# santiagolmedo/gnn_qot_estimation

Measured on AMD Instinct MI355X. Metric: graphs/sec (train step) on 100-node/400-edge synthetic topologies, batch=1024, higher is better.
Workload: dtype f32; 1 GPU; configs[1]: 2-layer TopologicalGNN (TransformerConv+NNConv) hidden=64, 100-node/400-directed-edge topologies, batch=1024 graphs per GPU, dropout 0.5, SGD momentum 0.9, SmoothL1; CSR build included in every step; graphs_per_gpu=1024, global_batch=1024, distinct_graphs_per_gpu=1024, launch=hip-graph replay, 4 whole steps (fwd+bwd+optimizer each) per graph, steps_per_graph=4, collective_in_graph=False, parallelism=dp1, prime_steps=45, collective_world_size=1, all_reduce_floats=68715

## Files before the change

gnn_qot_estimation_amd/csrc/nnconv_mfma.hip:

```cpp
#include "common.hpp"
#include "mfma_tile.hpp"
#include "nnconv_finalize_dev.hpp"
#include "split_bf16.hpp"

namespace qot {

template <int D, bool TRANSPOSE>
__device__ __forceinline__ void nnconv_gather_tile(
    float* __restrict__ At, const float* __restrict__ x, int ldx, const float* __restrict__ ea,
    const float* __restrict__ w1, const float* __restrict__ b1, const int32_t* __restrict__ rowptr,
    const int32_t* __restrict__ col, const int32_t* __restrict__ eidx, const float* __restrict__ invdeg,
    int64_t tile0, int64_t N, float4& root0, float4& root1) {
    constexpr int K = 2 * D;
    const int sub = threadIdx.x & 7, il = threadIdx.x >> 3;
    const int c0 = 8 * sub;
    const int64_t i = tile0 + il;
    float4 acc0[K + 1], acc1[K + 1];
    root0 = f4zero(); root1 = f4zero();
    int beg = 0, end = 0;
    float srow = 0.f;
    if (i < N) {
        beg = rowptr[i]; end = rowptr[i + 1];
        if (!TRANSPOSE) srow = invdeg[i];
        root0 = ld4(x + i * ldx + c0);
        root1 = ld4(x + i * ldx + c0 + 4);
    }
    const int own = (i < N) ? (int)i : 0;
#define QOT_ACC(FIRSTSLOT, H, X, A) ((FIRSTSLOT) ? scale4((H), (X)) : fma4((H), (X), (A)))
#define QOT_EDGE4(U0, FIRST)                                                                            \
        {                                                                                               \
            float4 xa[4], xb[4];                                                                        \
            float sc[4];                                                                                \
            int jj[4];                                                                                  \
            jj[0] = group8_bcast<U0 + 0>(myj); jj[1] = group8_bcast<U0 + 1>(myj);                       \
            jj[2] = group8_bcast<U0 + 2>(myj); jj[3] = group8_bcast<U0 + 3>(myj);                       \
            sc[0] = group8_bcast<U0 + 0>(mysc); sc[1] = group8_bcast<U0 + 1>(mysc);                     \
            sc[2] = group8_bcast<U0 + 2>(mysc); sc[3] = group8_bcast<U0 + 3>(mysc);                     \
            _Pragma("unroll") for (int u = 0; u < 4; ++u) {                                             \
                const float* xr = x + (int64_t)jj[u] * ldx + c0;                                        \
                xa[u] = ld4(xr);                                                                        \
                xb[u] = ld4(xr + 4);                                                                    \
            }                                                                                           \
            _Pragma("unroll") for (int kk = 0; kk < K; ++kk) {                                          \
                const float h0 = group8_bcast<U0 + 0>(myh[kk]), h1 = group8_bcast<U0 + 1>(myh[kk]);     \
                acc0[kk] = QOT_ACC(FIRST, h0, xa[0], acc0[kk]); acc1[kk] = QOT_ACC(FIRST, h0, xb[0], acc1[kk]); \
                acc0[kk] = fma4(h1, xa[1], acc0[kk]); acc1[kk] = fma4(h1, xb[1], acc1[kk]);             \
            }                                                                                           \
            acc0[K] = QOT_ACC(FIRST, sc[0], xa[0], acc0[K]); acc1[K] = QOT_ACC(FIRST, sc[0], xb[0], acc1[K]); \
            acc0[K] = fma4(sc[1], xa[1], acc0[K]); acc1[K] = fma4(sc[1], xb[1], acc1[K]);               \
             \
             \
            if (cnt > U0 + 2) {                                                                         \
                _Pragma("unroll") for (int kk = 0; kk < K; ++kk) {                                      \
                    const float h2 = group8_bcast<U0 + 2>(myh[kk]), h3 = group8_bcast<U0 + 3>(myh[kk]); \
                    acc0[kk] = fma4(h2, xa[2], acc0[kk]); acc1[kk] = fma4(h2, xb[2], acc1[kk]);         \
                    acc0[kk] = fma4(h3, xa[3], acc0[kk]); acc1[kk] = fma4(h3, xb[3], acc1[kk]);         \
                }                                                                                       \
                _Pragma("unroll") for (int u = 2; u < 4; ++u) {                                         \
                    acc0[K] = fma4(sc[u], xa[u], acc0[K]);                                              \
                    acc1[K] = fma4(sc[u], xb[u], acc1[K]);                                              \
                }                                                                                       \
            }                                                                                           \
        }
#define QOT_FWD_BATCH(FIRST)                                                                            \
    {                                                                                                   \
        const int p = base + sub;                                                                       \
        int myj = own;                                                                                  \
        float myh[K], mysc = 0.f;                                                                       \
        _Pragma("unroll") for (int kk = 0; kk < K; ++kk) myh[kk] = 0.f;                                 \
        if (p < end) {                                                                                  \
            myj = col[p];                                                                               \
            const int64_t e = (int64_t)eidx[p];                                                         \
            float ee[D];                                                                                \
            _Pragma("unroll") for (int d = 0; d < D; ++d) ee[d] = ea[e * D + d];                        \
            mysc = TRANSPOSE ? invdeg[myj] : srow;                                                      \
            _Pragma("unroll") for (int kk = 0; kk < K; ++kk) {                                          \
                float h = b1[kk];                                                                       \
                _Pragma("unroll") for (int d = 0; d < D; ++d) h = fmaf(w1[kk * D + d], ee[d], h);       \
                myh[kk] = fmaxf(h, 0.f) * mysc;                                                         \
            }                                                                                           \
        }                                                                                               \
        const int cnt = (end - base < 8) ? end - base : 8;                                              \
        QOT_EDGE4(0, FIRST)                                                                             \
        if (cnt > 4) QOT_EDGE4(4, false)                                                                \
    }
    int base = beg;
    QOT_FWD_BATCH(true)
    for (base = beg + 8; base < end; base += 8) QOT_FWD_BATCH(false)
#undef QOT_FWD_BATCH
#undef QOT_EDGE4
#undef QOT_ACC
    float4* At4 = reinterpret_cast<float4*>(At);
#pragma unroll
    for (int kk = 0; kk <= K; ++kk) {
        const int g = kk * 8 + sub;
        At4[at4_slot(g, 0, il)] = make_float4(acc0[kk].x, acc0[kk].z, acc1[kk].x, acc1[kk].z);
        At4[at4_slot(g, 1, il)] = make_float4(acc0[kk].y, acc0[kk].w, acc1[kk].y, acc1[kk].w);
    }
}

template <int D, bool TRANSPOSE, bool SPLIT = false>
__global__ __launch_bounds__(256, 2) void nnconv_mfma64_kernel(
    const float* __restrict__ x, int ldx, const float* __restrict__ ea, const float* __restrict__ w1,
    const float* __restrict__ b1, const int32_t* __restrict__ rowptr, const int32_t* __restrict__ col,
    const int32_t* __restrict__ eidx, const float* __restrict__ invdeg, const float* __restrict__ Wp,
    const float* __restrict__ bias, float* __restrict__ out, int64_t N, ActParams act,
    const u32x4* __restrict__ Ws = nullptr, int64_t ws_planes = 0) {
    static_assert(!SPLIT || !TRANSPOSE, "split form: forward only");
    constexpr int K = 2 * D;
    constexpr int KM = (K + 1) * 64;
    constexpr int GM = KM / 16;
    constexpr int CH = 4;
    __shared__ __attribute__((aligned(16))) float At[KM * 32];
    const int64_t ntiles = (N + 31) / 32;
    const float bz = bias ? bias[((threadIdx.x >> 6) & 1) * 32 + (threadIdx.x & 31)] : 0.f;
    const uint64_t drop_step = (act.enabled && act.thr16) ? (uint64_t)act.step[0] : 0;
#pragma unroll 1
    for (int64_t it = 0;; ++it) {
    const int64_t tile = xcd_tile(it, ntiles);
    if (tile < 0) break;
    const int64_t tile0 = tile * 32;
    float4 root0, root1;
    nnconv_gather_tile<D, TRANSPOSE>(At, x, ldx, ea, w1, b1, rowptr, col, eidx, invdeg, tile0, N, root0, root1);
    const float4* At4 = reinterpret_cast<const float4*>(At);
    const int lane = threadIdx.x & 63, wave = threadIdx.x >> 6;
    const int nh = wave & 1, kh = wave >> 1;
    const int r31 = lane & 31, hi = lane >> 5;
    f32x16 c;
#pragma unroll
    for (int r = 0; r < 16; ++r) c[r] = 0.f;
    if constexpr (SPLIT) {
        constexpr int ST = (K + 2) * 64 / 16;
        constexpr int SM = GM / 2;
        constexpr int SC = 2;
        constexpr int NCS = SM / SC;
        constexpr int NBS = 3;
        static_assert(GM % 4 == 0, "chunking");
        const u32x4* wsn = Ws + (int64_t)nh * ST * 64 + lane;
        const u32x4* wsp = wsn + (int64_t)kh * SM * 64;
        const u32x4* rsp = wsn + (int64_t)(2 * SM + 2 * kh) * 64;
        asm volatile("" : "+v"(rsp));
        Bf3 rbs[2];
#pragma unroll
        for (int u = 0; u < 2; ++u) rbs[u] = load_split_b(rsp + u * 64, ws_planes);
        Bf3 sb[NBS][SC];
#pragma unroll
        for (int q = 0; q < NBS - 1; ++q)
#pragma unroll
            for (int u = 0; u < SC; ++u) sb[q][u] = load_split_b(wsp + (q * SC + u) * 64, ws_planes);
        lds_barrier();
        int ch = 0;
#pragma unroll 1
        for (; ch + NBS <= NCS; ch += NBS) {
#pragma unroll
            for (int q = 0; q < NBS; ++q) {
                if (ch + q + NBS - 1 < NCS) {
#pragma unroll
                    for (int u = 0; u < SC; ++u)
                        sb[(q + NBS - 1) % NBS][u] = load_split_b(wsp + ((ch + q + NBS - 1) * SC + u) * 64, ws_planes);
                }
#pragma unroll
                for (int u = 0; u < SC; ++u) c = mfma_split_step(At4, kh * GM + 2 * ((ch + q) * SC + u), hi, r31, sb[q][u], c);
            }
        }
#pragma unroll
        for (int q = 0; q < NBS - 1; ++q) {
            if (ch + q < NCS) {
#pragma unroll
                for (int u = 0; u < SC; ++u) c = mfma_split_step(At4, kh * GM + 2 * ((ch + q) * SC + u), hi, r31, sb[q][u], c);
            }
        }
        lds_barrier();
        {
            float4* At4w = reinterpret_cast<float4*>(At);
            const int sub = threadIdx.x & 7, il = threadIdx.x >> 3;
            At4w[at4_slot(sub, 0, il)] = make_float4(root0.x, root0.z, root1.x, root1.z);
            At4w[at4_slot(sub, 1, il)] = make_float4(root0.y, root0.w, root1.y, root1.w);
        }
        __syncthreads();
#pragma unroll
        for (int u = 0; u < 2; ++u) c = mfma_split_step(At4, kh * 4 + 2 * u, hi, r31, rbs[u], c);
    } else {
    const float4* wpn = reinterpret_cast<const float4*>(Wp) + (int64_t)nh * (2 * GM + 8) * 64 + lane;
    const float4* wp = wpn + (int64_t)kh * GM * 64;
    const float4* rbp = wpn + (int64_t)(2 * GM + kh * 4) * 64;
    asm volatile("" : "+v"(rbp));
    float4 rb[4];
#pragma unroll
    for (int u = 0; u < 4; ++u) rb[u] = rbp[u * 64];
    constexpr int NCH = GM / CH;
    constexpr int NB = 4;
    float4 bb[NB][CH];
#pragma unroll
    for (int q = 0; q < NB - 1; ++q)
#pragma unroll
        for (int u = 0; u < CH; ++u) bb[q][u] = wp[(q * CH + u) * 64];
    lds_barrier();
    int ch = 0;
#pragma unroll 1
    for (; ch + NB <= NCH; ch += NB) {
#pragma unroll
        for (int q = 0; q < NB; ++q) {
            if (ch + q + NB - 1 < NCH) {
#pragma unroll
                for (int u = 0; u < CH; ++u) bb[(q + NB - 1) % NB][u] = wp[((ch + q + NB - 1) * CH + u) * 64];
            }
#pragma unroll
            for (int u = 0; u < CH; ++u) c = mfma_group(At4, kh * GM + (ch + q) * CH + u, hi, r31, bb[q][u], c);
        }
    }
#pragma unroll
    for (int q = 0; q < NB - 1; ++q) {
        if (ch + q < NCH) {
#pragma unroll
            for (int u = 0; u < CH; ++u) c = mfma_group(At4, kh * GM + (ch + q) * CH + u, hi, r31, bb[q][u], c);
        }
    }
    lds_barrier();
    {
        float4* At4 = reinterpret_cast<float4*>(At);
        const int sub = threadIdx.x & 7, il = threadIdx.x >> 3;
        At4[at4_slot(sub, 0, il)] = make_float4(root0.x, root0.z, root1.x, root1.z);
        At4[at4_slot(sub, 1, il)] = make_float4(root0.y, root0.w, root1.y, root1.w);
    }
    __syncthreads();
#pragma unroll
    for (int u = 0; u < 4; ++u) c = mfma_group(At4, kh * 4 + u, hi, r31, rb[u], c);
    }
    float* red = At + 64 * 32;
    if (kh) {
#pragma unroll
        for (int r = 0; r < 8; ++r) red[((2 + nh) * 8 + r) * 64 + lane] = c[r];
    } else {
#pragma unroll
        for (int r = 0; r < 8; ++r) red[(nh * 8 + r) * 64 + lane] = c[8 + r];
    }
    lds_barrier();
    {
        const int colg = nh * 32 + r31;
        float v[8];
        if (kh) {
#pragma unroll
            for (int r = 0; r < 8; ++r) v[r] = c[8 + r] + red[(nh * 8 + r) * 64 + lane] + bz;
        } else {
#pragma unroll
            for (int r = 0; r < 8; ++r) v[r] = c[r] + red[((2 + nh) * 8 + r) * 64 + lane] + bz;
        }
        uint32_t zlo[8], zhi[8];
        const bool drop = act.enabled && act.thr16;
        if (drop) {
            const int jq = r31 & 3;
            uint32_t mylo[2], myhi[2];
#pragma unroll
            for (int t = 0; t < 2; ++t) {
                const int rr = kh * 8 + 2 * jq + t;
                const int row = (rr & 3) + 8 * (rr >> 2) + 4 * hi;
                const uint64_t flat = (uint64_t)((tile0 + row) * 64 + colg);
                const uint64_t z = act_hash64(act.seed, drop_step, flat >> 2);
                mylo[t] = (uint32_t)z; myhi[t] = (uint32_t)(z >> 32);
            }
#define QOT_ZSHARE(S)                                                                                   \
            zlo[2 * (S)] = __builtin_amdgcn_update_dpp(0, mylo[0], (S) * 0x55, 0xF, 0xF, true);         \
            zhi[2 * (S)] = __builtin_amdgcn_update_dpp(0, myhi[0], (S) * 0x55, 0xF, 0xF, true);         \
            zlo[2 * (S) + 1] = __builtin_amdgcn_update_dpp(0, mylo[1], (S) * 0x55, 0xF, 0xF, true);     \
            zhi[2 * (S) + 1] = __builtin_amdgcn_update_dpp(0, myhi[1], (S) * 0x55, 0xF, 0xF, true);
            QOT_ZSHARE(0) QOT_ZSHARE(1) QOT_ZSHARE(2) QOT_ZSHARE(3)
#undef QOT_ZSHARE
        }
#pragma unroll
        for (int r = 0; r < 8; ++r) {
            const int rr = kh * 8 + r;
            const int row = (rr & 3) + 8 * (rr >> 2) + 4 * hi;
            const int64_t i = tile0 + row;
            float y = v[r];
            if (act.enabled) {
                y = y > 0.f ? y : act.slope * y;
                if (drop) {
                    const uint64_t z = ((uint64_t)zhi[r] << 32) | zlo[r];
                    const bool keep = ((uint32_t)(z >> (16 * (colg & 3))) & 0xFFFFu) >= act.thr16;
                    y = keep ? y * act.keep_scale : 0.f;
                }
            }
            if (i < N) out[i * 64 + colg] = y;
        }
    }
    lds_barrier();
    }
}


template <int D, bool SPLIT>
__global__ __launch_bounds__(512, 2) void nnconv_adjoint_dw64_kernel(
    const float* __restrict__ g, int ldg, const float* __restrict__ xf, int ldx, const float* __restrict__ ea,
    const float* __restrict__ w1, const float* __restrict__ b1, const int32_t* __restrict__ rowptr_t,
    const int32_t* __restrict__ col_t, const int32_t* __restrict__ eid_t, const float* __restrict__ invdeg,
    const float* __restrict__ Wp, float* __restrict__ gx, float* __restrict__ slabs, int64_t N) {
    constexpr int K = 2 * D;
    constexpr int KT = (K + 2) * 64;
    constexpr int GQ = KT / 8 / 4;
    constexpr int MB = KT / 32;
    constexpr int TPW = MB * 2 / 8;
    static_assert(GQ % 4 == 0 || GQ % 5 == 0, "chunking");
    constexpr int CH = (GQ % 4 == 0) ? 4 : 5;
    __shared__ __attribute__((aligned(16))) float Ut[KT * 32];
    __shared__ __attribute__((aligned(16))) float red[8 * 3 * 4 * 64];
    __shared__ __attribute__((aligned(16))) float xs[32 * 64];
    float4* Ut4 = reinterpret_cast<float4*>(Ut);
    const int lane = threadIdx.x & 63, wave = threadIdx.x >> 6;
    const int r31 = lane & 31, hi = lane >> 5;
    const int nh = wave & 1, kq = wave >> 1;
    const int ah = wave & 1, mb0 = wave >> 1;
    const int64_t ntiles = (N + 31) / 32;

    f32x16 dw[TPW];
#pragma unroll
    for (int t = 0; t < TPW; ++t)
#pragma unroll
        for (int r = 0; r < 16; ++r) dw[t][r] = 0.f;
    int dwoff[4];
    {
        const int kcol = mb0 * 32 + r31;
        const int gg = kcol >> 3, within = kcol & 7;
        const int base0 = ((2 * gg + (within & 1)) * 32) * 4 + (within >> 1);
        const int m = gg & 7;
#pragma unroll
        for (int b = 0; b < 4; ++b) dwoff[b] = base0 + ((((b ^ (m >> 1)) << 1) | (hi ^ (m & 1))) << 2);
    }
    const float4* wp = reinterpret_cast<const float4*>(Wp) + ((int64_t)nh * (KT / 8) + kq * GQ) * 64 + lane;

#pragma unroll 1
    for (int64_t it = 0;; ++it) {
        const int64_t tile = xcd_tile(it, ntiles);
        if (tile < 0) break;
        const int64_t tile0 = tile * 32;
        float4 xown;
        {
            const int64_t j = tile0 + (threadIdx.x >> 4);
            xown = (j < N) ? ld4(xf + j * ldx + 4 * (threadIdx.x & 15)) : f4zero();
        }
        {
            const int sub = threadIdx.x & 15, il = threadIdx.x >> 4;
            const int c0 = 4 * sub;
            const int64_t j = tile0 + il;
            float4 acc[K + 2];
            acc[K + 1] = f4zero();
            int beg = 0, end = 0;
            if (j < N) { beg = rowptr_t[j]; end = rowptr_t[j + 1]; acc[K + 1] = ld4(g + j * ldg + c0); }
            const int own = (j < N) ? (int)j : 0;
#define QOT_ADJ_EDGE(U)                                                                                  \
                {                                                                                        \
                    const int64_t i = (int64_t)row16_bcast<U>(myi);                                      \
                    gr[(U) & 3] = ld4(g + i * ldg + c0);                                                 \
                    sc[(U) & 3] = row16_bcast<U>(mysc);                                                  \
                }
#define QOT_ADJ_FMA(U, FIRSTSLOT)                                                                        \
                {                                                                                        \
                    _Pragma("unroll") for (int kk = 0; kk < K; ++kk)                                     \
                        acc[kk] = (FIRSTSLOT) ? scale4(row16_bcast<U>(myh[kk]), gr[(U) & 3])             \
                                              : fma4(row16_bcast<U>(myh[kk]), gr[(U) & 3], acc[kk]);     \
                    acc[K] = (FIRSTSLOT) ? scale4(sc[(U) & 3], gr[(U) & 3]) : fma4(sc[(U) & 3], gr[(U) & 3], acc[K]); \
                }
#define QOT_ADJ_EDGE4(U0, FIRST)                                                                         \
                {                                                                                        \
                    float4 gr[4];                                                                        \
                    float sc[4];                                                                         \
                    QOT_ADJ_EDGE(U0) QOT_ADJ_EDGE(U0 + 1) QOT_ADJ_EDGE(U0 + 2) QOT_ADJ_EDGE(U0 + 3)      \
                    QOT_ADJ_FMA(U0, FIRST) QOT_ADJ_FMA(U0 + 1, false)                                    \
                     \
                     \
                    if (cnt > U0 + 2) { QOT_ADJ_FMA(U0 + 2, false) QOT_ADJ_FMA(U0 + 3, false) }          \
                }
#define QOT_ADJ_BATCH(FIRST)                                                                             \
            {                                                                                            \
                const int p = base + sub;                                                                \
                int myi = own;                                                                           \
                float myh[K], mysc = 0.f;                                                                \
                _Pragma("unroll") for (int kk = 0; kk < K; ++kk) myh[kk] = 0.f;                          \
                if (p < end) {                                                                           \
                    myi = col_t[p];                                                                      \
                    const int64_t e = (int64_t)eid_t[p];                                                 \
                    float ee[D];                                                                         \
                    _Pragma("unroll") for (int d = 0; d < D; ++d) ee[d] = ea[e * D + d];                 \
                    mysc = invdeg[myi];                                                                  \
                    _Pragma("unroll") for (int kk = 0; kk < K; ++kk) {                                   \
                        float h = b1[kk];                                                                \
                        _Pragma("unroll") for (int d = 0; d < D; ++d) h = fmaf(w1[kk * D + d], ee[d], h); \
                        myh[kk] = fmaxf(h, 0.f) * mysc;                                                  \
                    }                                                                                    \
                }                                                                                        \
                const int cnt = (end - base < 16) ? end - base : 16;                                     \
                QOT_ADJ_EDGE4(0, FIRST)                                                                  \
                if (cnt > 4) QOT_ADJ_EDGE4(4, false)                                                     \
                if (cnt > 8) QOT_ADJ_EDGE4(8, false)                                                     \
                if (cnt > 12) QOT_ADJ_EDGE4(12, false)                                                   \
            }
            int base = beg;
            QOT_ADJ_BATCH(true)
            for (base = beg + 16; base < end; base += 16) QOT_ADJ_BATCH(false)
#undef QOT_ADJ_BATCH
#undef QOT_ADJ_EDGE4
#undef QOT_ADJ_FMA
#undef QOT_ADJ_EDGE
#pragma unroll
            for (int kk = 0; kk < K + 2; ++kk) {
                const int gg = kk * 8 + (sub >> 1);
                float2* s0 = reinterpret_cast<float2*>(&Ut4[at4_slot(gg, 0, il)]) + (sub & 1);
                float2* s1 = reinterpret_cast<float2*>(&Ut4[at4_slot(gg, 1, il)]) + (sub & 1);
                *s0 = make_float2(acc[kk].x, acc[kk].z);
                *s1 = make_float2(acc[kk].y, acc[kk].w);
            }
        }
        {
            const int sub = threadIdx.x & 15, il = threadIdx.x >> 4;
            *reinterpret_cast<float4*>(&xs[il * 64 + 4 * sub]) = xown;
        }
        constexpr int NCH = GQ / CH;
        float4 bc[CH], bn[CH];
#pragma unroll
        for (int u = 0; u < CH; ++u) bc[u] = wp[u * 64];
        lds_barrier();
        f32x16 c;
#pragma unroll
        for (int r = 0; r < 16; ++r) c[r] = 0.f;
        {
            int ch = 0;
#pragma unroll 1
            for (; ch + 1 < NCH; ch += 2) {
#pragma unroll
                for (int u = 0; u < CH; ++u) bn[u] = wp[((ch + 1) * CH + u) * 64];
#pragma unroll
                for (int u = 0; u < CH; ++u) c = mfma_group(Ut4, kq * GQ + ch * CH + u, hi, r31, bc[u], c);
                if (ch + 2 < NCH) {
#pragma unroll
                    for (int u = 0; u < CH; ++u) bc[u] = wp[((ch + 2) * CH + u) * 64];
                }
#pragma unroll
                for (int u = 0; u < CH; ++u) c = mfma_group(Ut4, kq * GQ + (ch + 1) * CH + u, hi, r31, bn[u], c);
            }
            if (NCH & 1) {
#pragma unroll
                for (int u = 0; u < CH; ++u) c = mfma_group(Ut4, kq * GQ + (NCH - 1) * CH + u, hi, r31, bc[u], c);
            }
        }
#define QOT_GIVE(OWNER, SLOT)                                                                        \
        _Pragma("unroll") for (int rr = 0; rr < 4; ++rr)                                             \
            red[((((OWNER) * 2 + nh) * 3 + (SLOT)) * 4 + rr) * 64 + lane] = c[4 * (OWNER) + rr];
        if (kq == 0) { QOT_GIVE(1, 0) QOT_GIVE(2, 0) QOT_GIVE(3, 0) }
        else if (kq == 1) { QOT_GIVE(0, 0) QOT_GIVE(2, 1) QOT_GIVE(3, 1) }
        else if (kq == 2) { QOT_GIVE(0, 1) QOT_GIVE(1, 1) QOT_GIVE(3, 2) }
        else { QOT_GIVE(0, 2) QOT_GIVE(1, 2) QOT_GIVE(2, 2) }
#undef QOT_GIVE
        if (SPLIT) {
#pragma unroll 1
            for (int s = 0; s < 2; ++s) {
                float xv[8];
#pragma unroll
                for (int j = 0; j < 8; ++j)
                    xv[j] = xs[(8 * (2 * s + (j >> 2)) + 2 * (j & 3) + hi) * 64 + ah * 32 + r31];
                const Bf3 xb = split8(make_float4(xv[0], xv[1], xv[2], xv[3]), make_float4(xv[4], xv[5], xv[6], xv[7]));
#pragma unroll
                for (int t = 0; t < TPW; ++t) {
                    float av[8];
#pragma unroll
                    for (int j = 0; j < 8; ++j) av[j] = Ut[dwoff[j & 3] + (2 * s + (j >> 2)) * 32 + t * 4096];
                    dw[t] = mfma_split6(
                        split8(make_float4(av[0], av[1], av[2], av[3]), make_float4(av[4], av[5], av[6], av[7])), xb, dw[t]);
                    __builtin_amdgcn_sched_barrier(0);
                }
            }
        } else {
            float abuf[2][TPW], xbuf[2];
            const float* xsl = xs + hi * 64 + ah * 32 + r31;
#pragma unroll
            for (int t = 0; t < TPW; ++t) abuf[0][t] = Ut[dwoff[0] + t * 4096];
            xbuf[0] = xsl[0];
#pragma unroll
            for (int sidx = 0; sidx < 16; ++sidx) {
                const int cur = sidx & 1;
                if (sidx + 1 < 16) {
                    const int sn = sidx + 1;
#pragma unroll
                    for (int t = 0; t < TPW; ++t) abuf[cur ^ 1][t] = Ut[dwoff[sn & 3] + (sn >> 2) * 32 + t * 4096];
                    xbuf[cur ^ 1] = xsl[sn * 128];
                }
                __builtin_amdgcn_sched_barrier(0);
#pragma unroll
                for (int t = 0; t < TPW; ++t)
                    dw[t] = __builtin_amdgcn_mfma_f32_32x32x2f32(abuf[cur][t], xbuf[cur], dw[t], 0, 0, 0);
                __builtin_amdgcn_sched_barrier(0);
            }
        }
        lds_barrier();
        {
            float v[4];
            if (kq == 0) { v[0] = c[0]; v[1] = c[1]; v[2] = c[2]; v[3] = c[3]; }
            else if (kq == 1) { v[0] = c[4]; v[1] = c[5]; v[2] = c[6]; v[3] = c[7]; }
            else if (kq == 2) { v[0] = c[8]; v[1] = c[9]; v[2] = c[10]; v[3] = c[11]; }
            else { v[0] = c[12]; v[1] = c[13]; v[2] = c[14]; v[3] = c[15]; }
            const int colg = nh * 32 + r31;
#pragma unroll
            for (int rr = 0; rr < 4; ++rr) {
#pragma unroll
                for (int slot = 0; slot < 3; ++slot) v[rr] += red[(((kq * 2 + nh) * 3 + slot) * 4 + rr) * 64 + lane];
                const int reg = 4 * kq + rr;
                const int row = (reg & 3) + 8 * (reg >> 2) + 4 * hi;
                const int64_t j = tile0 + row;
                if (j < N) gx[j * 64 + colg] = v[rr];
            }
        }
        lds_barrier();
    }
    float* slab = slabs + (int64_t)blockIdx.x * KT * 64;
#pragma unroll
    for (int t = 0; t < TPW; ++t)
#pragma unroll
        for (int r = 0; r < 16; ++r) {
            const int row = (r & 3) + 8 * (r >> 2) + 4 * hi;
            slab[((mb0 + 4 * t) * 32 + row) * 64 + ah * 32 + r31] = dw[t][r];
        }
}

__global__ void adj_slab_reduce_kernel(const float* __restrict__ slabs, int nslabs, int per_group, int64_t elems,
                                       int64_t slab_stride, float* __restrict__ dst, int64_t dst_stride) {
    int64_t t = blockIdx.x * (int64_t)blockDim.x + threadIdx.x;
    if (t * 4 >= elems) return;
    const int s0 = blockIdx.y * per_group;
    int s1 = s0 + per_group;
    if (s1 > nslabs) s1 = nslabs;
    float4 acc = f4zero();
    int sidx = s0;
    for (; sidx + 8 <= s1; sidx += 8) {
        float4 v[8];
#pragma unroll
        for (int u = 0; u < 8; ++u) v[u] = ld4(slabs + (int64_t)(sidx + u) * slab_stride + 4 * t);
#pragma unroll
        for (int u = 0; u < 8; ++u) acc = add4(acc, v[u]);
    }
    for (; sidx < s1; ++sidx) acc = add4(acc, ld4(slabs + (int64_t)sidx * slab_stride + 4 * t));
    st4(dst + blockIdx.y * dst_stride + 4 * t, acc);
}

__global__ void adj_slab_final_params_kernel(const float* __restrict__ slabs, int nslabs, int64_t elems,
                                             int64_t slab_stride, float* __restrict__ dst, int K) {
    int64_t t = blockIdx.x * (int64_t)blockDim.x + threadIdx.x;
    if (t * 4 >= elems) return;
    float4 acc = f4zero();
    for (int sidx = 0; sidx < nslabs; ++sidx) acc = add4(acc, ld4(slabs + (int64_t)sidx * slab_stride + 4 * t));
    const int64_t e = 4 * t;
    const int a0 = (int)(e & 63), o = (int)((e >> 6) & 63), kb = (int)(e >> 12);
    const float v[4] = {acc.x, acc.y, acc.z, acc.w};
#pragma unroll
    for (int c = 0; c < 4; ++c) {
        const int a = a0 + c;
        int64_t idx;
        if (kb < K) idx = ((int64_t)a * 64 + o) * K + kb;
        else if (kb == K) idx = (int64_t)4096 * K + a * 64 + o;
        else idx = (int64_t)4096 * (K + 1) + o * 64 + a;
        dst[idx] = v[c];
    }
}

__global__ void gradh_partial_sum_kernel(const float* __restrict__ partials, int nblk, int n, int KD,
                                         float* __restrict__ gw1, float* __restrict__ gb1) {
    const int t = blockIdx.x * (blockDim.x >> 6) + (threadIdx.x >> 6);
    if (t >= n) return;
    const float s = wave_sum_partials(partials, nblk, n, t);
    if ((threadIdx.x & 63) == 0) { if (t < KD) gw1[t] = s; else gb1[t - KD] = s; }
}

}

using namespace qot;

int qot_nnconv_gen_launch(const float* x, int ld_x, const float* edge_attr, const float* w1, const float* b1,
                          const int32_t* rowptr, const int32_t* col, const int32_t* edge_ids, const float* invdeg,
                          int transpose, const float* w_perm, const float* bias, float* out, int64_t N, int H, int D,
                          const ActParams& ap, hipStream_t stream);
int qot_nnconv_gradh_gen_launch(const float* grad_out, int ld_g, const float* x, int ld_x, const float* edge_attr,
                                const float* w1, const float* b1, const int32_t* rowptr, const int32_t* col,
                                const int32_t* eid, const float* invdeg, const float* b_perm, float* gw1, float* gb1,
                                float* workspace, int64_t N, int H, int D, hipStream_t stream);

extern "C" int qot_nnconv_fused(const float* x, int ld_x, const float* edge_attr, const float* w1,
                                const float* b1, const int32_t* rowptr, const int32_t* col,
                                const int32_t* edge_ids, const float* invdeg, int transpose,
                                const float* w_perm, const float* bias, float* out, int64_t N, int H, int D,
                                int act, float act_slope, float act_p, uint64_t act_seed,
                                const int64_t* act_step, qot_stream_t stream) {
    if (N < 0 || !rowptr) return QOT_ERR_BADARG;
    if (H != 16 && H != 32 && H != 64 && H != 128 && H != 256) return QOT_ERR_UNSUPPORTED;
    if (N == 0) return QOT_OK;
    if (!x || !w1 || !b1 || !invdeg || !w_perm || !out || (ld_x & 3)) return QOT_ERR_BADARG;
    if (H != 64 || transpose == 2 || transpose == 3) {
        if (D > 4) return QOT_ERR_UNSUPPORTED;
        return qot_nnconv_gen_launch(x, ld_x, edge_attr, w1, b1, rowptr, col, edge_ids, invdeg, transpose & 1, w_perm,
                                     bias, out, N, H, D, make_act(act, act_slope, act_p, act_seed, act_step),
                                     (hipStream_t)stream);
    }
    int grid = grid_for(N, 32);
    if (grid > 2 * num_cus()) grid = 2 * num_cus();
    const ActParams ap = make_act(act, act_slope, act_p, act_seed, act_step);
    QOT_DISPATCH_D(D, {
        if (transpose)
            nnconv_mfma64_kernel<kD, true><<<grid, 256, 0, (hipStream_t)stream>>>(
                x, ld_x, edge_attr, w1, b1, rowptr, col, edge_ids, invdeg, w_perm, bias, out, N, ap);
        else
            nnconv_mfma64_kernel<kD, false><<<grid, 256, 0, (hipStream_t)stream>>>(
                x, ld_x, edge_attr, w1, b1, rowptr, col, edge_ids, invdeg, w_perm, bias, out, N, ap);
    });
    QOT_LAUNCH_CHECK();
    return QOT_OK;
}

extern "C" int qot_nnconv_fused_split(const float* x, int ld_x, const float* edge_attr, const float* w1,
                                      const float* b1, const int32_t* rowptr, const int32_t* col,
                                      const int32_t* edge_ids, const float* invdeg, const void* w_split,
                                      int64_t split_stride, const float* bias, float* out, int64_t N, int H, int D,
                                      int act, float act_slope, float act_p, uint64_t act_seed,
                                      const int64_t* act_step, qot_stream_t stream) {
    if (N < 0 || !rowptr) return QOT_ERR_BADARG;
    if (H != 64 || D > 4) return QOT_ERR_UNSUPPORTED;
    if (N == 0) return QOT_OK;
    if (!x || !w1 || !b1 || !invdeg || !w_split || !out || (ld_x & 3) || ((uintptr_t)w_split & 15) || (split_stride & 7) ||
        split_stride < (int64_t)(2 * D + 2) * 4096)
        return QOT_ERR_BADARG;
    int grid = grid_for(N, 32);
    if (grid > 2 * num_cus()) grid = 2 * num_cus();
    const ActParams ap = make_act(act, act_slope, act_p, act_seed, act_step);
    QOT_DISPATCH_D(D, {
        if (kD <= 4)
            nnconv_mfma64_kernel<(kD <= 4 ? kD : 4), false, true><<<grid, 256, 0, (hipStream_t)stream>>>(
                x, ld_x, edge_attr, w1, b1, rowptr, col, edge_ids, invdeg, nullptr, bias, out, N, ap,
                static_cast<const u32x4*>(w_split), split_stride / 8);
    });
    QOT_LAUNCH_CHECK();
    return QOT_OK;
}

int qot_nnconv_gradh64_launch(const float* grad_out, int ld_g, const float* x, int ld_x, const float* edge_attr, const float* w1,
                              const float* b1, const int32_t* rowptr, const int32_t* col, const int32_t* eid, const float* invdeg,
                              const float* b_perm, const void* b_split, int64_t split_stride, float* workspace, int64_t N, int D,
                              int grid, hipStream_t stream);
extern "C" size_t qot_nnconv_gradh_workspace_floats(int D) {
    return (size_t)2 * 256 * 2 * (size_t)(2 * D * (D + 1));
}

static int nnconv_gradh_impl(const float* grad_out, int ld_g, const float* x, int ld_x,
                             const float* edge_attr, const float* w1, const float* b1,
                             const int32_t* rowptr, const int32_t* col, const int32_t* eid,
                             const float* invdeg, const float* b_perm, const void* b_split, int64_t split_stride,
                             float* gw1, float* gb1,
                             float* workspace, int64_t N, int H, int D, qot_stream_t stream_) {
    hipStream_t stream = (hipStream_t)stream_;
    if (N < 0 || !rowptr) return QOT_ERR_BADARG;
    if ((H != 16 && H != 32 && H != 64 && H != 128 && H != 256) || D > 4) return QOT_ERR_UNSUPPORTED;
    if (!grad_out || !x || !w1 || !b1 || !invdeg || !(b_perm || b_split) || (!gw1 != !gb1) || !workspace || (ld_g & 3) ||
        (ld_x & 3) || ((uintptr_t)b_split & 15) || (b_split && ((split_stride & 7) || split_stride < (int64_t)2 * D * 64 * 64)))
        return QOT_ERR_BADARG;
    if (b_split && H != 64) return QOT_ERR_UNSUPPORTED;
    if (!gw1 && H != 64) return QOT_ERR_UNSUPPORTED;
    if (H != 64)
        return qot_nnconv_gradh_gen_launch(grad_out, ld_g, x, ld_x, edge_attr, w1, b1, rowptr, col, eid, invdeg, b_perm,
                                           gw1, gb1, workspace, N, H, D, stream);
    int grid = grid_for(N > 0 ? N : 1, 32);
    if (grid > 2 * num_cus()) grid = 2 * num_cus();
    const int K = 2 * D;
    const int rc = qot_nnconv_gradh64_launch(grad_out, ld_g, x, ld_x, edge_attr, w1, b1, rowptr, col, eid, invdeg, b_perm,
                                             b_split, split_stride, workspace, N, D, grid, stream);
    if (rc != QOT_OK) return rc;
    QOT_LAUNCH_CHECK();
    if (!gw1) return QOT_OK;
    const int n = K * (D + 1);
    gradh_partial_sum_kernel<<<grid_for(n, 4), 256, 0, stream>>>(workspace, grid, n, K * D, gw1, gb1);
    QOT_LAUNCH_CHECK();
    return QOT_OK;
}

extern "C" int qot_nnconv_gradh_fused(const float* grad_out, int ld_g, const float* x, int ld_x,
                                      const float* edge_attr, const float* w1, const float* b1,
                                      const int32_t* rowptr, const int32_t* col, const int32_t* eid,
                                      const float* invdeg, const float* b_perm, float* gw1, float* gb1,
                                      float* workspace, int64_t N, int H, int D, qot_stream_t stream) {
    return nnconv_gradh_impl(grad_out, ld_g, x, ld_x, edge_attr, w1, b1, rowptr, col, eid, invdeg, b_perm, nullptr, 0, gw1, gb1,
                             workspace, N, H, D, stream);
}

extern "C" int qot_nnconv_gradh_split(const float* grad_out, int ld_g, const float* x, int ld_x,
                                      const float* edge_attr, const float* w1, const float* b1,
                                      const int32_t* rowptr, const int32_t* col, const int32_t* eid,
                                      const float* invdeg, const void* b_split, int64_t split_stride, float* gw1, float* gb1,
                                      float* workspace, int64_t N, int H, int D, qot_stream_t stream) {
    if (!b_split) return QOT_ERR_BADARG;
    return nnconv_gradh_impl(grad_out, ld_g, x, ld_x, edge_attr, w1, b1, rowptr, col, eid, invdeg, nullptr, b_split, split_stride,
                             gw1, gb1,
                             workspace, N, H, D, stream);
}

extern "C" int qot_nnconv_bwd_finalize(const float* adj_workspace, const float* gradh_workspace, float* grad_params,
                                       float* gw1, float* gb1, int64_t N, int H, int D, qot_stream_t stream_) {
    if (N <= 0 || H != 64 || D < 1 || D > 4) return (H != 64 || D > 4) ? QOT_ERR_UNSUPPORTED : QOT_ERR_BADARG;
    qot_role_t r{};
    r.kind = QOT_ROLE_NNCONV_FINALIZE64;
    r.p[0] = adj_workspace; r.p[1] = gradh_workspace; r.p[2] = grad_params; r.p[3] = gw1; r.p[4] = gb1;
    r.i[0] = N; r.i[1] = D;
    return qot_run_roles(&r, 1, stream_);
}

extern "C" size_t qot_nnconv_adjoint_dw_workspace_floats(int D) {
    return (size_t)(num_cus() > 256 ? num_cus() : 256) * kAdjBlocksPerCu * (size_t)((2 * D + 2) * 64) * 64;
}

extern "C" int qot_nnconv_adjoint_dw(const float* grad_out, int ld_g, const float* x, int ld_x,
                                     const float* edge_attr, const float* w1, const float* b1,
                                     const int32_t* rowptr_t, const int32_t* col_t, const int32_t* eid_t,
                                     const float* invdeg, const float* w_perm, float* grad_x, float* gwcat_t,
                                     int param_layout, float* workspace, int64_t N, int H, int D,
                                     qot_stream_t stream_) {
    hipStream_t stream = (hipStream_t)stream_;
    if (N <= 0 || !rowptr_t) return QOT_ERR_BADARG;
    if (H != 64 || D > 4) return QOT_ERR_UNSUPPORTED;
    if (!grad_out || !x || !w1 || !b1 || !invdeg || !w_perm || !grad_x || !gwcat_t || !workspace || (ld_g & 3))
        return QOT_ERR_BADARG;
    int grid = grid_for(N, 32);
    const int cap = num_cus() * kAdjBlocksPerCu;
    if (grid > cap) grid = cap;
    const char* f32_env = getenv("QOT_NNCONV_F32_MFMA");
    const bool f32_mfma = f32_env && f32_env[0] == '1' && f32_env[1] == '\0';
    QOT_DISPATCH_D(D, {
        if (kD <= 4) {
            constexpr int kD4 = kD <= 4 ? kD : 4;
            if (f32_mfma)
                nnconv_adjoint_dw64_kernel<kD4, false><<<grid, 512, 0, stream>>>(
                    grad_out, ld_g, x, ld_x, edge_attr, w1, b1, rowptr_t, col_t, eid_t, invdeg, w_perm, grad_x,
                    workspace, N);
            else
                nnconv_adjoint_dw64_kernel<kD4, true><<<grid, 512, 0, stream>>>(
                    grad_out, ld_g, x, ld_x, edge_attr, w1, b1, rowptr_t, col_t, eid_t, invdeg, w_perm, grad_x,
                    workspace, N);
        }
    });
    QOT_LAUNCH_CHECK();
    if (param_layout == 2) return QOT_OK;
    const int64_t elems = (int64_t)(2 * D + 2) * 64 * 64;
    const int per_group = 16;
    const int groups = (grid + per_group - 1) / per_group;
    adj_slab_reduce_kernel<<<dim3(grid_for(elems / 4, 256), groups), 256, 0, stream>>>(
        workspace, grid, per_group, elems, elems, workspace, (int64_t)per_group * elems);
    QOT_LAUNCH_CHECK();
    if (param_layout)
        adj_slab_final_params_kernel<<<grid_for(elems / 4, 256), 256, 0, stream>>>(
            workspace, groups, elems, (int64_t)per_group * elems, gwcat_t, 2 * D);
    else
        adj_slab_reduce_kernel<<<dim3(grid_for(elems / 4, 256), 1), 256, 0, stream>>>(
            workspace, groups, groups, elems, (int64_t)per_group * elems, gwcat_t, 0);
    QOT_LAUNCH_CHECK();
    return QOT_OK;
}
```

Baseline: 2.484 million graphs/s.

## Add 64-row NNConv forward kernel reusing split-bf16 weight loads across two tiles

Adds a new NNConv forward kernel that processes two 32-row tiles per work unit. Each weight fragment loaded through a register ring feeds MFMAs for both tiles, and the gather is done in two column-half passes with 4 lanes per row, using DPP quad broadcasts to share edge data. Work is distributed per XCD chunk, and the new kernel is the default path, with an env var to fall back to the old 32-row kernel. This amortizes weight traffic and barrier costs, at the price of more registers, more LDS, fewer blocks for small N, and extra code complexity.

```diff
diff --git a/gnn_qot_estimation_amd/csrc/nnconv_fwd64.hip b/gnn_qot_estimation_amd/csrc/nnconv_fwd64.hip
--- /dev/null
+++ b/gnn_qot_estimation_amd/csrc/nnconv_fwd64.hip
@@ -0,0 +1,300 @@
+#include "common.hpp"
+#include "mfma_tile.hpp"
+#include "split_bf16.hpp"
+
+namespace qot {
+
+__device__ __forceinline__ int at4_slot64(int lg, int hi, int i) { return (2 * lg + hi) * 64 + (i ^ (2 * (lg & 3))); }
+
+template <int SRC>
+__device__ __forceinline__ int quad_bcast(int v) {
+    return __builtin_amdgcn_update_dpp(0, v, SRC * 0x55, 0xF, 0xF, true);
+}
+template <int SRC>
+__device__ __forceinline__ float quad_bcast(float v) { return dpp_move<SRC * 0x55>(v); }
+
+struct Walk64 {
+    int64_t ubeg;
+    int slot, P, full_rounds, n2, n1;
+};
+__device__ __forceinline__ Walk64 walk64_init(int64_t nunits) {
+    Walk64 w;
+    int64_t cnt;
+    if ((int)gridDim.x % 8 != 0) {
+        w.slot = blockIdx.x; w.P = gridDim.x; w.ubeg = 0; cnt = nunits;
+    } else {
+        const int xcd = blockIdx.x % 8;
+        w.slot = blockIdx.x / 8; w.P = gridDim.x / 8;
+        const int64_t chunk = (nunits + 7) / 8;
+        w.ubeg = xcd * chunk;
+        cnt = nunits - w.ubeg;
+        cnt = cnt < 0 ? 0 : (cnt > chunk ? chunk : cnt);
+    }
+    w.full_rounds = (int)(cnt / (2 * w.P));
+    const int rem = (int)(cnt - (int64_t)w.full_rounds * 2 * w.P);
+    w.n2 = rem > w.P ? rem - w.P : 0;
+    w.n1 = rem - 2 * w.n2;
+    return w;
+}
+__device__ __forceinline__ int walk64_tile(const Walk64& w, int it, int64_t& unit) {
+    if (it < w.full_rounds) { unit = w.ubeg + ((int64_t)it * w.P + w.slot) * 2; return 64; }
+    if (it > w.full_rounds) return 0;
+    const int64_t base = w.ubeg + (int64_t)w.full_rounds * 2 * w.P;
+    if (w.slot < w.n2) { unit = base + 2 * w.slot; return 64; }
+    if (w.slot < w.n2 + w.n1) { unit = base + 2 * w.n2 + (w.slot - w.n2); return 32; }
+    return 0;
+}
+
+template <int D>
+__device__ __forceinline__ void nnconv_gather_pass64(
+    float* __restrict__ At, const float* __restrict__ x, int ldx, const float* __restrict__ ea,
+    const float* __restrict__ w1, const float* __restrict__ b1, const int32_t* __restrict__ rowptr,
+    const int32_t* __restrict__ col, const int32_t* __restrict__ eidx, const float* __restrict__ invdeg,
+    int64_t row0, int nrows, int64_t N, int cb, float4& root0, float4& root1) {
+    constexpr int K = 2 * D;
+    const int sub = threadIdx.x & 3, il = threadIdx.x >> 2;
+    const int c0 = cb + 8 * sub;
+    const int64_t i = row0 + il;
+    const bool live = il < nrows && i < N;
+    float4 acc0[K + 1], acc1[K + 1];
+    root0 = f4zero(); root1 = f4zero();
+    int beg = 0, end = 0;
+    float srow = 0.f;
+    if (live) {
+        beg = rowptr[i]; end = rowptr[i + 1];
+        srow = invdeg[i];
+        root0 = ld4(x + i * ldx + c0);
+        root1 = ld4(x + i * ldx + c0 + 4);
+    }
+    const int own = live ? (int)i : 0;
+#define QOT_ACC(FIRSTSLOT, H, X, A) ((FIRSTSLOT) ? scale4((H), (X)) : fma4((H), (X), (A)))
+#define QOT_EDGE4(SET, FIRST)                                                                           \
+        {                                                                                               \
+            float4 xa[4], xb[4];                                                                        \
+            float sc[4];                                                                                \
+            int jj[4];                                                                                  \
+            jj[0] = quad_bcast<0>(myj[SET]); jj[1] = quad_bcast<1>(myj[SET]);                           \
+            jj[2] = quad_bcast<2>(myj[SET]); jj[3] = quad_bcast<3>(myj[SET]);                           \
+            sc[0] = quad_bcast<0>(mysc[SET]); sc[1] = quad_bcast<1>(mysc[SET]);                         \
+            sc[2] = quad_bcast<2>(mysc[SET]); sc[3] = quad_bcast<3>(mysc[SET]);                         \
+            _Pragma("unroll") for (int u = 0; u < 4; ++u) {                                             \
+                const float* xr = x + (int64_t)jj[u] * ldx + c0;                                        \
+                xa[u] = ld4(xr);                                                                        \
+                xb[u] = ld4(xr + 4);                                                                    \
+            }                                                                                           \
+            _Pragma("unroll") for (int kk = 0; kk < K; ++kk) {                                          \
+                const float h0 = quad_bcast<0>(myh[SET][kk]), h1 = quad_bcast<1>(myh[SET][kk]);         \
+                acc0[kk] = QOT_ACC(FIRST, h0, xa[0], acc0[kk]); acc1[kk] = QOT_ACC(FIRST, h0, xb[0], acc1[kk]); \
+                acc0[kk] = fma4(h1, xa[1], acc0[kk]); acc1[kk] = fma4(h1, xb[1], acc1[kk]);             \
+            }                                                                                           \
+            acc0[K] = QOT_ACC(FIRST, sc[0], xa[0], acc0[K]); acc1[K] = QOT_ACC(FIRST, sc[0], xb[0], acc1[K]); \
+            acc0[K] = fma4(sc[1], xa[1], acc0[K]); acc1[K] = fma4(sc[1], xb[1], acc1[K]);               \
+                                     \
+            if (cnt > 4 * (SET) + 2) {                                                                  \
+                _Pragma("unroll") for (int kk = 0; kk < K; ++kk) {                                      \
+                    const float h2 = quad_bcast<2>(myh[SET][kk]), h3 = quad_bcast<3>(myh[SET][kk]);     \
+                    acc0[kk] = fma4(h2, xa[2], acc0[kk]); acc1[kk] = fma4(h2, xb[2], acc1[kk]);         \
+                    acc0[kk] = fma4(h3, xa[3], acc0[kk]); acc1[kk] = fma4(h3, xb[3], acc1[kk]);         \
+                }                                                                                       \
+                _Pragma("unroll") for (int u = 2; u < 4; ++u) {                                         \
+                    acc0[K] = fma4(sc[u], xa[u], acc0[K]);                                              \
+                    acc1[K] = fma4(sc[u], xb[u], acc1[K]);                                              \
+                }                                                                                       \
+            }                                                                                           \
+        }
+#define QOT_FWD_BATCH(FIRST)                                                                            \
+    {                                                                                                   \
+        int myj[2];                                                                                     \
+        float myh[2][K], mysc[2];                                                                       \
+        _Pragma("unroll") for (int t = 0; t < 2; ++t) {                                                 \
+            const int p = base + 4 * t + sub;                                                           \
+            myj[t] = own; mysc[t] = 0.f;                                                                \
+            _Pragma("unroll") for (int kk = 0; kk < K; ++kk) myh[t][kk] = 0.f;                          \
+            if (p < end) {                                                                              \
+                myj[t] = col[p];                                                                        \
+                const int64_t e = (int64_t)eidx[p];                                                     \
+                float ee[D];                                                                            \
+                _Pragma("unroll") for (int d = 0; d < D; ++d) ee[d] = ea[e * D + d];                    \
+                mysc[t] = srow;                                                                         \
+                _Pragma("unroll") for (int kk = 0; kk < K; ++kk) {                                      \
+                    float h = b1[kk];                                                                   \
+                    _Pragma("unroll") for (int d = 0; d < D; ++d) h = fmaf(w1[kk * D + d], ee[d], h);   \
+                    myh[t][kk] = fmaxf(h, 0.f) * srow;                                                  \
+                }                                                                                       \
+            }                                                                                           \
+        }                                                                                               \
+        const int cnt = (end - base < 8) ? end - base : 8;                                              \
+        QOT_EDGE4(0, FIRST)                                                                             \
+        if (cnt > 4) QOT_EDGE4(1, false)                                                                \
+    }
+    int base = beg;
+    QOT_FWD_BATCH(true)
+    for (base = beg + 8; base < end; base += 8) QOT_FWD_BATCH(false)
+#undef QOT_FWD_BATCH
+#undef QOT_EDGE4
+#undef QOT_ACC
+    float4* At4 = reinterpret_cast<float4*>(At);
+#pragma unroll
+    for (int kk = 0; kk <= K; ++kk) {
+        const int lg = kk * 4 + sub;
+        At4[at4_slot64(lg, 0, il)] = make_float4(acc0[kk].x, acc0[kk].z, acc1[kk].x, acc1[kk].z);
+        At4[at4_slot64(lg, 1, il)] = make_float4(acc0[kk].y, acc0[kk].w, acc1[kk].y, acc1[kk].w);
+    }
+}
+
+__device__ __forceinline__ void nnconv_fwd64_finish(const f32x16& c, const float* __restrict__ red, float* __restrict__ out,
+                                                    int64_t rowb, int64_t N, const ActParams& act, uint64_t drop_step,
+                                                    float bz, int nh, int kh, int lane) {
+    const int r31 = lane & 31, hi = lane >> 5;
+    const int colg = nh * 32 + r31;
+    float v[8];
+    if (kh) {
+#pragma unroll
+        for (int r = 0; r < 8; ++r) v[r] = c[8 + r] + red[(nh * 8 + r) * 64 + lane] + bz;
+    } else {
+#pragma unroll
+        for (int r = 0; r < 8; ++r) v[r] = c[r] + red[((2 + nh) * 8 + r) * 64 + lane] + bz;
+    }
+    uint32_t zlo[8], zhi[8];
+    const bool drop = act.enabled && act.thr16;
+    if (drop) {
+        const int jq = r31 & 3;
+        uint32_t mylo[2], myhi[2];
+#pragma unroll
+        for (int t = 0; t < 2; ++t) {
+            const int rr = kh * 8 + 2 * jq + t;
+            const int row = (rr & 3) + 8 * (rr >> 2) + 4 * hi;
+            const uint64_t flat = (uint64_t)((rowb + row) * 64 + colg);
+            const uint64_t z = act_hash64(act.seed, drop_step, flat >> 2);
+            mylo[t] = (uint32_t)z; myhi[t] = (uint32_t)(z >> 32);
+        }
+#define QOT_ZSHARE(S)                                                                                   \
+        zlo[2 * (S)] = __builtin_amdgcn_update_dpp(0, mylo[0], (S) * 0x55, 0xF, 0xF, true);             \
+        zhi[2 * (S)] = __builtin_amdgcn_update_dpp(0, myhi[0], (S) * 0x55, 0xF, 0xF, true);             \
+        zlo[2 * (S) + 1] = __builtin_amdgcn_update_dpp(0, mylo[1], (S) * 0x55, 0xF, 0xF, true);         \
+        zhi[2 * (S) + 1] = __builtin_amdgcn_update_dpp(0, myhi[1], (S) * 0x55, 0xF, 0xF, true);
+        QOT_ZSHARE(0) QOT_ZSHARE(1) QOT_ZSHARE(2) QOT_ZSHARE(3)
+#undef QOT_ZSHARE
+    }
+#pragma unroll
+    for (int r = 0; r < 8; ++r) {
+        const int rr = kh * 8 + r;
+        const int row = (rr & 3) + 8 * (rr >> 2) + 4 * hi;
+        const int64_t i = rowb + row;
+        float y = v[r];
+        if (act.enabled) {
+            y = y > 0.f ? y : act.slope * y;
+            if (drop) {
+                const uint64_t z = ((uint64_t)zhi[r] << 32) | zlo[r];
+                const bool keep = ((uint32_t)(z >> (16 * (colg & 3))) & 0xFFFFu) >= act.thr16;
+                y = keep ? y * act.keep_scale : 0.f;
+            }
+        }
+        if (i < N) out[i * 64 + colg] = y;
+    }
+}
+
+constexpr int kRing = 4;
+
+template <int D>
+__global__ __launch_bounds__(256, 2) void nnconv_fwd64_kernel(
+    const float* __restrict__ x, int ldx, const float* __restrict__ ea, const float* __restrict__ w1,
+    const float* __restrict__ b1, const int32_t* __restrict__ rowptr, const int32_t* __restrict__ col,
+    const int32_t* __restrict__ eidx, const float* __restrict__ invdeg, const float* __restrict__ bias,
+    float* __restrict__ out, int64_t N, ActParams act, const u32x4* __restrict__ Ws, int64_t ws_planes) {
+    constexpr int K = 2 * D;
+    constexpr int NS = K + 2;
+    constexpr int ST = (K + 2) * 4;
+    __shared__ __attribute__((aligned(16))) float At[64 * (K + 1) * 32];
+    const int lane = threadIdx.x & 63, wave = threadIdx.x >> 6;
+    const int nh = wave & 1, kh = wave >> 1;
+    const int r31 = lane & 31, hi = lane >> 5;
+    const float bz = bias ? bias[nh * 32 + r31] : 0.f;
+    const uint64_t drop_step = (act.enabled && act.thr16) ? (uint64_t)act.step[0] : 0;
+    const float4* At4 = reinterpret_cast<const float4*>(At);
+    const int a0 = at4_slot64(2 * kh, hi, r31), a1 = at4_slot64(2 * kh + 1, hi, r31);
+    const u32x4* wsw = Ws + ((int64_t)nh * ST + kh) * 64 + lane;
+    const Walk64 walk = walk64_init((N + 31) / 32);
+#pragma unroll 1
+    for (int it = 0;; ++it) {
+        int64_t unit = 0;
+        const int nrows = walk64_tile(walk, it, unit);
+        if (nrows == 0) break;
+        const int64_t row0 = unit * 32;
+        const bool full = nrows == 64 && row0 + 32 < N;
+        f32x16 c0, c1;
+#pragma unroll
+        for (int r = 0; r < 16; ++r) { c0[r] = 0.f; c1[r] = 0.f; }
+#pragma unroll 1
+        for (int p = 0; p < 2; ++p) {
+            float4 root0, root1;
+            nnconv_gather_pass64<D>(At, x, ldx, ea, w1, b1, rowptr, col, eidx, invdeg, row0, nrows, N, 32 * p, root0, root1);
+            int woff = p * 128;
+            asm volatile("" : "+v"(woff));
+            const u32x4* wsp = wsw + woff;
+            Bf3 ring[kRing];
+#pragma unroll
+            for (int j = 0; j < kRing - 1; ++j)
+                if (j < NS) ring[j] = load_split_b(wsp + j * 256, ws_planes);
+            lds_barrier();
+#pragma unroll
+            for (int j = 0; j < NS; ++j) {
+                if (j + kRing - 1 < NS) ring[(j + kRing - 1) % kRing] = load_split_b(wsp + (j + kRing - 1) * 256, ws_planes);
+                if (j == NS - 1) {
+                    lds_barrier();
+                    float4* At4w = reinterpret_cast<float4*>(At);
+                    const int sub = threadIdx.x & 3, il = threadIdx.x >> 2;
+                    At4w[at4_slot64(sub, 0, il)] = make_float4(root0.x, root0.z, root1.x, root1.z);
+                    At4w[at4_slot64(sub, 1, il)] = make_float4(root0.y, root0.w, root1.y, root1.w);
+                    lds_barrier();
+                }
+                const int blk = (j == NS - 1 ? 0 : j) * 512;
+                c0 = mfma_split6(split8(At4[a0 + blk], At4[a1 + blk]), ring[j % kRing], c0);
+                if (full) c1 = mfma_split6(split8(At4[a0 + blk + 32], At4[a1 + blk + 32]), ring[j % kRing], c1);
+            }
+            if (p == 0) lds_barrier();
+        }
+        float* red = At + 4 * 2 * 64 * 4;
+        if (kh) {
+#pragma unroll
+            for (int r = 0; r < 8; ++r) red[((2 + nh) * 8 + r) * 64 + lane] = c0[r];
+        } else {
+#pragma unroll
+            for (int r = 0; r < 8; ++r) red[(nh * 8 + r) * 64 + lane] = c0[8 + r];
+        }
+        if (full) {
+            if (kh) {
+#pragma unroll
+                for (int r = 0; r < 8; ++r) red[2048 + ((2 + nh) * 8 + r) * 64 + lane] = c1[r];
+            } else {
+#pragma unroll
+                for (int r = 0; r < 8; ++r) red[2048 + (nh * 8 + r) * 64 + lane] = c1[8 + r];
+            }
+        }
+        lds_barrier();
+        nnconv_fwd64_finish(c0, red, out, row0, N, act, drop_step, bz, nh, kh, lane);
+        if (full) nnconv_fwd64_finish(c1, red + 2048, out, row0 + 32, N, act, drop_step, bz, nh, kh, lane);
+        lds_barrier();
+    }
+}
+
+}
+
+using namespace qot;
+
+int qot_nnconv_fwd64_launch(const float* x, int ld_x, const float* edge_attr, const float* w1, const float* b1,
+                            const int32_t* rowptr, const int32_t* col, const int32_t* edge_ids, const float* invdeg,
+                            const void* w_split, int64_t split_stride, const float* bias, float* out, int64_t N, int D,
+                            const ActParams& ap, hipStream_t stream) {
+    int grid = grid_for(N, 64);
+    if (grid > 2 * num_cus()) grid = 2 * num_cus();
+    QOT_DISPATCH_D(D, {
+        if (kD <= 4)
+            nnconv_fwd64_kernel<(kD <= 4 ? kD : 4)><<<grid, 256, 0, stream>>>(
+                x, ld_x, edge_attr, w1, b1, rowptr, col, edge_ids, invdeg, bias, out, N, ap,
+                static_cast<const u32x4*>(w_split), split_stride / 8);
+        else
+            return QOT_ERR_UNSUPPORTED;
+    });
+    return QOT_OK;
+}
diff --git a/gnn_qot_estimation_amd/csrc/nnconv_mfma.hip b/gnn_qot_estimation_amd/csrc/nnconv_mfma.hip
--- a/gnn_qot_estimation_amd/csrc/nnconv_mfma.hip
+++ b/gnn_qot_estimation_amd/csrc/nnconv_mfma.hip
@@ -612,6 +612,11 @@
     return QOT_OK;
 }
 
+int qot_nnconv_fwd64_launch(const float* x, int ld_x, const float* edge_attr, const float* w1, const float* b1,
+                            const int32_t* rowptr, const int32_t* col, const int32_t* edge_ids, const float* invdeg,
+                            const void* w_split, int64_t split_stride, const float* bias, float* out, int64_t N, int D,
+                            const ActParams& ap, hipStream_t stream);
+
 extern "C" int qot_nnconv_fused_split(const float* x, int ld_x, const float* edge_attr, const float* w1,
                                       const float* b1, const int32_t* rowptr, const int32_t* col,
                                       const int32_t* edge_ids, const float* invdeg, const void* w_split,
@@ -624,9 +629,17 @@
     if (!x || !w1 || !b1 || !invdeg || !w_split || !out || (ld_x & 3) || ((uintptr_t)w_split & 15) || (split_stride & 7) ||
         split_stride < (int64_t)(2 * D + 2) * 4096)
         return QOT_ERR_BADARG;
+    const ActParams ap = make_act(act, act_slope, act_p, act_seed, act_step);
+    const char* t32_env = getenv("QOT_NNCONV_FWD_TILE32");
+    if (!(t32_env && t32_env[0] == '1' && t32_env[1] == '\0')) {
+        const int rc = qot_nnconv_fwd64_launch(x, ld_x, edge_attr, w1, b1, rowptr, col, edge_ids, invdeg, w_split, split_stride,
+                                               bias, out, N, D, ap, (hipStream_t)stream);
+        if (rc != QOT_OK) return rc;
+        QOT_LAUNCH_CHECK();
+        return QOT_OK;
+    }
     int grid = grid_for(N, 32);
     if (grid > 2 * num_cus()) grid = 2 * num_cus();
-    const ActParams ap = make_act(act, act_slope, act_p, act_seed, act_step);
     QOT_DISPATCH_D(D, {
         if (kD <= 4)
             nnconv_mfma64_kernel<(kD <= 4 ? kD : 4), false, true><<<grid, 256, 0, (hipStream_t)stream>>>(
```

New measurement: 2.454 million graphs/s. 0.988x the previous value.
